# DaanVrancken/HubbardTN

Measured on AMD Instinct MI355X. Metric: DMRG sweep time (s) + GS energy/site, 1-band Hubbard L=64 chi=1024, lower is better.
Workload: dtype c128; 1 GPU; one-band Hubbard chain L=64 U/t=4, half filling, fZ2xSU(2)xU(1), two-site DMRG sweep (2L-3=125 bond updates) at chi=1024 (TensorKit dim units); model=one_band, L=64, chi=1024, krylovdim=30, parallelism=sector-parallel apply x1, backend=hip

## Files before the change

### hubbardtn_amd/csrc/htn_backend_hip.hip

```cpp
#include <dlfcn.h>

#include <map>
#include <mutex>

#include "htn_common.h"
#include "htn_core.h"

namespace {

__global__ __launch_bounds__(256) void k_scale_z(double2* __restrict__ x, int64_t n, double f) {
    for (int64_t j = (int64_t)blockIdx.x * blockDim.x + threadIdx.x; j < n; j += (int64_t)gridDim.x * blockDim.x) {
        const double2 v = x[j];
        x[j] = make_double2(v.x * f, v.y * f);
    }
}

__global__ __launch_bounds__(256) void k_copy_words(uint32_t* __restrict__ dst, const uint32_t* __restrict__ src, size_t n) {
    for (size_t j = (size_t)blockIdx.x * blockDim.x + threadIdx.x; j < n; j += (size_t)gridDim.x * blockDim.x) dst[j] = src[j];
    __threadfence_system();
}

struct Rccl {
    void* lib = nullptr;
    int (*GetUniqueId)(void*) = nullptr;
// ... 225 lines not shown
        if (nvec > 32) return htn::set_error("orthonormalise_rows: more than 32 rows");
        if (ensure_lan_scratch(htn_dots_scratch_elems(32) + 64)) return 1;
        double2* P = (double2*)Pv;
        double2* part = (double2*)lan_scratch;
        double2* coef = part + htn_dots_scratch_elems(32);
        double2* nrm = coef + 32;
        int k = 0;
        for (int r = 0; r < nvec; ++r) {
            double2* dst = P + (int64_t)k * n;
            if (r != k) HIP_TRY(hipMemcpyAsync(dst, P + (int64_t)r * n, sizeof(double2) * n, hipMemcpyDeviceToDevice, st));
            if (htn_dots_z(dst, n, 1, dst, n, nrm, part, st)) return 1;
            for (int pass = 0; pass < 2 && k > 0; ++pass) {
                if (htn_dots_z(P, n, k, dst, n, coef, part, st)) return 1;
                if (htn_axpys_z(dst, P, n, k, coef, -1.0, n, st)) return 1;
            }
            if (htn_dots_z(dst, n, 1, dst, n, nrm + 1, part, st)) return 1;
            double h[4];
            if (download(h, nrm, sizeof(h))) return 1;
            const double n0 = h[0], n1 = h[2];
            if (!(n0 > 0.0) || !(n1 > drop_tol * drop_tol * n0)) continue;
            if (htn_scale_inv_sqrt_z(dst, dst, nrm + 1, n, st)) return 1;
            ++k;
        }
        *kept = k;
        return 0;
    }
    int jacobi_svd(void* G, void* Vj, double* S, const htn_svd_block* desc_dev, const htn_svd_block* desc_host, int n_blocks,
                   int max_m, int max_sweeps, double tol, int32_t* info_dev, const htn_svd_opts* opts) override {
        fork_open = true;
        const int rc = htn_jacobi_svd_z(G, Vj, S, desc_dev, desc_host, n_blocks, max_m, max_sweeps, tol, info_dev, opts, st);
        fork_open = false;
        return rc;
    }
    int qr_blocks(void* A, void* R, const htn_qr_block* desc_dev, const htn_qr_block* desc_host, int n_blocks) override {
        return htn_qr_blocks_z(A, R, desc_dev, desc_host, n_blocks, st);
    }
    int block_trdots(const void* A, const void* B, const htn_trdot_item* items_dev, const htn_trdot_item* items_host, int n_items,
                     void* out, int n_out) override {
        (void)items_host;
        const int64_t need = htn_trdots_scratch_elems(n_items);
        if (need > trd_scratch_elems) {
            if (trd_scratch) HIP_TRY(hipFree(trd_scratch));
            trd_scratch = nullptr, trd_scratch_elems = 0;
            HIP_TRY(hipMalloc(&trd_scratch, sizeof(double2) * 2 * need));
            trd_scratch_elems = 2 * need;
            if (htn_debug_poison()) HIP_TRY(hipMemsetAsync(trd_scratch, 0xFF, sizeof(double2) * trd_scratch_elems, st));
        }
        return htn_block_trdots_z(A, B, items_dev, n_items, out, n_out, trd_scratch, st);
    }
    int batched_copy(void* dst, const void* src, const int32_t* idx, const double* scl, const htn_copy_item* items, int n_items,
                     double gscale) override {
        return htn_batched_copy_z(dst, src, idx, scl, items, n_items, gscale, st);
    }
    int scale(void* x, int64_t n, double f) override {
        if (n <= 0) return 0;
        const int grid = (int)std::min<int64_t>((n + 255) / 256, 2048);
        hipLaunchKernelGGL(k_scale_z, dim3(grid), dim3(256), 0, st, (double2*)x, n, f);
        HIP_TRY(hipGetLastError());
        return 0;
    }
    int set_comm(int rank, int world, const void* id) override {
        Rccl& r = rccl();
        if (!r.ok) return htn::set_error("htn_ctx_set_comm: librccl.so could not be loaded");
        if (comm) {
            r.CommDestroy(comm);
            comm = nullptr;
// ... 52 lines not shown
```

### hubbardtn_amd/csrc/htn_common.h

```cpp
#pragma once
#include <hip/hip_runtime.h>
#include <stdint.h>
#include <stdio.h>
#include <stdlib.h>
#include <string.h>

#include <map>
#include <memory>
#include <mutex>
#include <utility>

#include "hubbardtn_hip.h"

char* htn_err_buf();

static inline int htn_fail(const char* what, hipError_t e) {
    snprintf(htn_err_buf(), 512, "%s: %s", what, hipGetErrorString(e));
    return 1;
}
static inline int htn_fail_msg(const char* what) {
    snprintf(htn_err_buf(), 512, "%s", what);
    return 1;
}
#define fail htn_fail
// ... 5 lines not shown
    } while (0)

typedef double d4 __attribute__((ext_vector_type(4)));

static inline hipError_t htn_event_spin(hipEvent_t ev) {
    hipError_t e;
    while ((e = hipEventQuery(ev)) == hipErrorNotReady) __builtin_ia32_pause();
    return e;
}
static inline hipError_t htn_stream_spin(hipStream_t st) {
    static thread_local hipEvent_t evs[64] = {};
    int dev = 0;
    hipError_t e = hipGetDevice(&dev);
    if (e != hipSuccess) return e;
    if (dev < 0 || dev >= 64) return hipStreamSynchronize(st);
    if (!evs[dev] && (e = hipEventCreateWithFlags(&evs[dev], hipEventDisableTiming)) != hipSuccess) return e;
    if ((e = hipEventRecord(evs[dev], st)) != hipSuccess) return e;
    return htn_event_spin(evs[dev]);
}


static inline bool htn_env_flag(const char* name) {
    const char* v = getenv(name);
    return v && v[0] && v[0] != '0';
}
static inline bool htn_debug_poison() {
    static const bool on = htn_env_flag("HTN_DEBUG_POISON");
    return on;
}
static inline bool htn_debug_event_waits() {
    static const bool on = htn_env_flag("HTN_DEBUG_EVENT_WAITS");
    return on;
}

struct LanRecord {
    unsigned long long w[4];
};
__host__ __device__ __forceinline__ unsigned long long lan_rotl(unsigned long long x, int r) { return (x << r) | (x >> (64 - r)); }
__host__ __device__ __forceinline__ unsigned long long lan_check(unsigned long long w0, unsigned long long w1, unsigned long long w2,
                                                                 unsigned long long serial) {
    return serial ^ lan_rotl(w0, 13) ^ lan_rotl(w1, 29) ^ lan_rotl(w2, 47) ^ 0x9E3779B97F4A7C15ull;
}
#define HTN_DOT_BLOCKS 256
struct HtnGemmPublish {
    const double* norm_partial;
    const double2* c1;
    const double2* c2;
    LanRecord* rec_out;
    unsigned long long serial;
};
int htn_grouped_gemm_launch(const void* const* bufs_host, const htn_tile* tiles, int32_t n_tiles, const htn_seg* segs,
                            const HtnGemmPublish* pub, hipStream_t stream);

enum HtnBufKind {
    HTN_BUF_DEVICE,
    HTN_BUF_PINNED,
    HTN_BUF_MAPPED
};
struct HtnBuf {
    const HtnBufKind kind;
    const bool poison;
    void* p = nullptr;
    void* dev = nullptr;
    size_t cap = 0;
    explicit HtnBuf(HtnBufKind k, bool poison_new = true) : kind(k), poison(poison_new) {}
    HtnBuf(const HtnBuf&) = delete;
// ... 125 lines not shown
```

### hubbardtn_amd/csrc/htn_core.h

```cpp
#pragma once
#include <stdint.h>
#include <string.h>

#include <array>
#include <complex>
#include <memory>
#include <string>
#include <unordered_map>
#include <utility>
#include <vector>

#include "hubbardtn_hip.h"

namespace htn {

typedef std::complex<double> cplx;

enum { BUF_X = 0, BUF_Y, BUF_L, BUF_R, BUF_Z, BUF_S1, BUF_S2, BUF_AUX };

struct Sec {
    int32_t N, j;
};
inline bool operator<(const Sec& a, const Sec& b) { return a.N < b.N || (a.N == b.N && a.j < b.j); }
inline bool operator==(const Sec& a, const Sec& b) { return a.N == b.N && a.j == b.j; }
// ... 242 lines not shown
    bool has_cen = false;
    int64_t n_idx = 0;
};
void plan_finalize(const ThetaLayout& tl, const SvdPlan& sp, const std::vector<int>& keep, const SiteLayout& layA,
                   const SiteLayout& layB, bool right, int64_t offA, int64_t offB, FinalizePlan& out);

struct Backend {
    virtual ~Backend() {}
    virtual int kind() const = 0;
    virtual int activate() { return 0; }
    virtual void* alloc(size_t bytes) = 0;
    virtual void release(void* p) = 0;
    virtual int upload(void* dst, const void* src_host, size_t bytes) = 0;
    virtual int download(void* dst_host, const void* src, size_t bytes) = 0;
    virtual int zero(void* p, size_t bytes) = 0;
    virtual int sync() = 0;
    virtual int grouped_gemm(const void* const* bufs, const htn_tile* tiles, int32_t n_tiles, const htn_seg* segs) = 0;
    virtual int lanczos(const htn_gemm_launch* stages, int n_stages, int x_slot, int y_slot, void* V, int64_t n,
                        int krylovdim, double tol, int max_restart, int zero_y, htn_exchange2_fn exchange, void* user,
                        double* eig, int* n_matvec, double* residual, double* matvec_ms) = 0;
    virtual int lanczos_orth(const htn_gemm_launch* stages, int n_stages, int x_slot, int y_slot, void* V, int64_t n,
                             int krylovdim, double tol, int max_restart, int zero_y, htn_exchange2_fn exchange, void* user,
                             const void* Q, int n_frozen, double* eig, int* n_matvec, double* residual, double* matvec_ms);
    virtual int krylov_expm(const htn_gemm_launch* stages, int n_stages, int x_slot, int y_slot, void* V, int64_t n, int krylovdim,
                            double dt_re, double dt_im, double tol, int max_restart, int zero_y, htn_exchange2_fn exchange, void* user,
                            double* growth, double* alpha0, int* n_matvec, double* err, double* matvec_ms);
    virtual int orthonormalise_rows(void* P, int64_t n, int nvec, double drop_tol, int* kept);
    virtual int qr_blocks(void* A, void* R, const htn_qr_block* desc_dev, const htn_qr_block* desc_host, int n_blocks);
    virtual int block_trdots(const void* A, const void* B, const htn_trdot_item* items_dev, const htn_trdot_item* items_host,
                             int n_items, void* out, int n_out);
    virtual int jacobi_svd(void* G, void* Vj, double* S, const htn_svd_block* desc_dev, const htn_svd_block* desc_host,
                           int n_blocks, int max_m, int max_sweeps, double tol, int32_t* info_dev,
                           const htn_svd_opts* opts) = 0;
    virtual int batched_copy(void* dst, const void* src, const int32_t* idx, const double* scl,
                             const htn_copy_item* items_dev, int n_items, double gscale) = 0;
    virtual int scale(void* x, int64_t n, double f) = 0;
    virtual int set_comm(int rank, int world, const void* id) { return 1; }
    virtual bool has_comm() const { return false; }
    virtual int allreduce(void* y, int64_t n) { return 1; }
    bool timing = false;
};

void qr_blocks_host(cplx* A, cplx* R, const htn_qr_block* desc, int n_blocks);

int set_error(const char* fmt, ...);
char* err_buf();

}
```

### hubbardtn_amd/csrc/htn_engine.cpp

```cpp
#include <math.h>
#include <stdio.h>
#include <stdlib.h>

#include <algorithm>
#include <atomic>
#include <chrono>
#include <map>

#include "htn_core.h"
#include "htn_expm.h"

namespace htn {
Backend* make_backend(int backend, int device, void* stream);
}
using namespace htn;

namespace {
void tridiag_lowest_host(const std::vector<double>& alpha, const std::vector<double>& beta, double* eig, std::vector<double>& vec) {
    const int k = (int)alpha.size();
    auto count = [&](double x) {
        int cnt = 0;
        double d = 1.0;
        for (int i = 0; i < k; ++i) {
            d = (alpha[i] - x) - (i ? beta[i - 1] * beta[i - 1] / d : 0.0);
// ... 479 lines not shown
};
struct MeetC {
    std::vector<htn_trdot_item> items;
    DBufP items_dev;
};
struct OrthState {
    htn_mps* phi = nullptr;
    std::vector<OvlLayoutP> Llay, Rlay;
    std::vector<DView> Lbuf, Rbuf;
};
struct Solve {
    std::shared_ptr<ApplyC> ap;
    int64_t n = 0;
    double E = 0.0, res = 0.0, mv_ms = 0.0;
    int nmv = 0;
    double growth = 1.0;
};
struct BondWork {
    ThetaLayoutP tl;
    Solve sol;
    DView V, z, Qb;
    std::shared_ptr<SvdC> sc;
    DView G, Vj;
    DBufP S, idx;
    size_t s_elems = 0;
    std::vector<double> s_host;
    int jac_sweeps = 0;
    std::vector<int> lens, qd, counts;
    std::vector<std::vector<int>> order;
    std::vector<double> vals;
    double nrm = 0.0, tw = 0.0;
    BondP mid;
    double tA = 0.0, tB = 0.0, tC = 0.0, tD = 0.0;
};

}

struct htn_mps {
    std::atomic<int> refs{1};
    htn_ctx* ctx;
    htn_mpo* mpo_handle = nullptr;
    Backend* be;
    const Mpo* mpo;
    int L;
    std::vector<BondP> bonds;
    std::vector<SiteLayoutP> site_lay;
    std::vector<DView> site_buf;
    std::vector<EnvLayoutP> Llay, Rlay;
    std::vector<DView> Lbuf, Rbuf;
    std::unordered_map<std::string, std::shared_ptr<const void>> cache;
    int64_t hits = 0, misses = 0;
    double energy = 0.0;
    std::map<int, Spectrum> spectra;
    std::map<int, std::pair<std::pair<int, double>, double>> cut_hint;
    std::map<int, int> sweeps_hint;
    std::vector<int32_t> idx_host;
    std::vector<OrthState> orth;
    int orth_dropped = 0;
    int centre = 0;

    template <class T, class F>
    std::shared_ptr<T> cached(const std::string& key, F build) {
        auto it = cache.find(key);
        if (it != cache.end()) {
            ++hits;
            return std::const_pointer_cast<T>(std::static_pointer_cast<const T>(it->second));
// ... 61 lines not shown
        return cached<const ThetaLayout>(std::string("tl") + bl->key + "|" + br->key,
                                         [&] { return build_theta_layout(mpo->sym, bl, br); });
    }
    int gemm(const DevTasks& d, std::initializer_list<std::pair<int, const void*>> bufs) {
        if (d.ntiles == 0) return 0;
        if (ensure_ws(d.ws_slots)) return 1;
        const void* table[HTN_MAX_BUFS] = {nullptr};
        for (auto& kv : bufs) table[kv.first] = kv.second;
        table[HTN_BUF_WS] = ws.ptr();
        return be->grouped_gemm(table, d.tiles, d.ntiles, d.segs);
    }

    template <class C, class P>
    std::shared_ptr<C> compile2(std::shared_ptr<C> e, const P& p) {
        if (upload_tasks(p.t1, e->d1) || upload_tasks(p.t2, e->d2)) return nullptr;
        e->zsize = p.zsize;
        e->flops = p.t1.flops + p.t2.flops;
        return e;
    }
    int env_step(char side, int i);
    int left_env(int i) { return env_step('L', i); }
    int right_env(int i) { return env_step('R', i); }
    int ovl_step(char side, const htn_mps* ket, int i, const OvlLayoutP& inl, const DView& in, OvlLayoutP* outl, DView* out);
    int ovl_boundary(const htn_mps* ket, int b, OvlLayoutP* outl, DView* out);
    int ovl_project(const OrthState& o, int i, const ThetaLayout& tl, cplx* dst);
    int orth_attach(htn_mps* const* others, int n);
    void orth_detach();
    std::shared_ptr<ApplyC> compile_apply(ApplyPlan& p, bool deal_y);
    std::shared_ptr<ApplyC> make_apply(int i, const ThetaLayout& tl);
    std::shared_ptr<ApplyC> make_apply1(int i, const SiteLayout& lay);
    int apply_stages(const ApplyC& ap, const DView& L, const DView& R, const DView& z, htn_gemm_launch* stages);
    int apply_once(const ApplyC& ap, const DView& L, const DView& R, int64_t n, const void* x_host, void* y_host, bool exchange);
    int theta_into(int i, const ThetaLayout& tl, cplx* dst);
    int bond_solve(int i, bool optimise, const htn_sweep_opts& o, StageClock& clk, BondWork& w, const cplx* evolve_dt = nullptr);
    std::shared_ptr<SvdC> make_svd(int i, const ThetaLayout& tl, bool right);
    int bond_svd(int i, bool right, const htn_sweep_opts& o, BondWork& w);
    int bond_truncate(int i, const htn_sweep_opts& o, BondWork& w);
    int bond_finalise(int i, bool right, BondWork& w);
    int bond_advance(int i, bool right);
    void bond_spectrum(int i, const BondWork& w);
    void fill_stats(htn_bond_stats* st, int bond, int direction, const Solve& sol, int64_t env_elems, int jacobi_sweeps,
                    int64_t svd_flops, double trunc_weight, const StageClock& clk);
    int update_bond(int i, int direction, bool right, bool optimise, const htn_sweep_opts& o, htn_bond_stats* st,
                    const cplx* evolve_dt = nullptr, double* log_growth = nullptr);
    int sweep(const htn_sweep_opts& o, htn_bond_stats* st, double* E);
    int evolve_checks(const htn_sweep_opts& o, const char* who) const;
    int evolve_site(int i, cplx dt, const htn_sweep_opts& o, htn_bond_stats* st, double* log_growth);
    int tdvp2_sweep(cplx dt, const htn_sweep_opts& o, htn_bond_stats* st, double* E, double* log_norm);
    int set_mpo(htn_mpo* m);
    int relay(const SiteLayout& from, const cplx* src, const SiteLayout& to, cplx* dst);
    int update_site(int i, int direction, bool optimise, const htn_sweep_opts& o, htn_bond_stats* st);
    int sweep1(const htn_sweep_opts& o, htn_bond_stats* st, double* E);
    int correlator(const htn_corr_channel& ch, cplx* out_host, double* norm_host);
};

int htn_mps::env_step(char side, int i) {
    const bool left = side == 'L';
    const SiteLayout& lay = *site_lay[i];
    if (lay.kind != side)
        return left ? set_error("left_env: site %d is not in left layout", i) : set_error("right_env: site %d is not in right layout", i);
    const MpoSite& W = mpo->sites[i];
    const int from = left ? i : i + 1, to = left ? i + 1 : i;
    std::vector<EnvLayoutP>& elay = left ? Llay : Rlay;
    std::vector<DView>& ebuf = left ? Lbuf : Rbuf;
    auto c = cached<EnvC>(ikey(left ? "lenv" : "renv", i) + bonds[i]->key + "|" + bonds[i + 1]->key, [&]() -> std::shared_ptr<EnvC> {
        auto e = std::make_shared<EnvC>();
        e->lay = build_env_layout(mpo->sym, side, bonds[to], left ? W.right : W.left);
// ... 161 lines not shown

static int exchange_tramp(void* y, int64_t n, void* user) {
    htn_ctx* ctx = (htn_ctx*)user;
    if (ctx->exch) return ctx->exch(y, n, ctx->exch_user);
    return ctx->be->allreduce(y, n);
}

int htn_mps::apply_once(const ApplyC& ap, const DView& L, const DView& R, int64_t n, const void* x_host, void* y_host, bool exchange) {
    DView x = zalloc(n, false), y = zalloc(n, true), z = zalloc(ap.zsize, false);
    if (!x.base || !y.base || !z.base) return set_error("device allocation failed");
    if (be->upload(x.ptr(), x_host, sizeof(cplx) * n)) return 1;
    if (ap.has_z && gemm(ap.dz, {{BUF_X, x.ptr()}, {BUF_L, L.ptr()}, {BUF_Z, z.ptr()}})) return 1;
    if (gemm(ap.dy, {{BUF_X, x.ptr()}, {BUF_Y, y.ptr()}, {BUF_L, L.ptr()}, {BUF_R, R.ptr()}, {BUF_Z, z.ptr()}})) return 1;
    if (exchange && exchange_tramp(y.ptr(), n, ctx)) return set_error("htn_heff2_apply: exchange failed");
    return be->download(y_host, y.ptr(), sizeof(cplx) * n);
}

void htn_mps::fill_stats(htn_bond_stats* st, int bond, int direction, const Solve& sol, int64_t env_elems, int jacobi_sweeps,
                         int64_t svd_flops, double trunc_weight, const StageClock& clk) {
    memset(st, 0, sizeof(*st));
    st->bond = bond, st->direction = direction;
    st->n_matvec = sol.nmv, st->jacobi_sweeps = jacobi_sweeps;
    st->chi_full = (int32_t)bonds[bond]->dim_full(mpo->sym), st->multiplets = bonds[bond]->multiplets();
    st->n_tiles = sol.ap->ntiles, st->n_segs = sol.ap->nsegs;
    st->theta_size = sol.n;
    st->apply_flops = sol.ap->flops, st->apply_bytes = 16 * (2 * sol.n + env_elems), st->svd_flops = svd_flops;
    st->energy = sol.E, st->residual = sol.res, st->trunc_weight = trunc_weight;
    st->t_plan = clk.plan, st->t_lanczos = clk.lanczos, st->t_env = clk.env;
    st->t_total = now() - clk.t0;
    st->t_svd = clk.svd >= 0.0 ? clk.svd : st->t_total - clk.plan - clk.lanczos - clk.env;
    st->matvec_ms = sol.mv_ms > 0.0 ? sol.mv_ms : 0.0;
}

int htn_mps::bond_solve(int i, bool optimise, const htn_sweep_opts& o, StageClock& clk, BondWork& w, const cplx* evolve_dt) {
    w.tl = theta_layout(bonds[i], bonds[i + 2]);
    const ThetaLayout& tl = *w.tl;
    Solve& s = w.sol;
    const int64_t n = s.n = tl.size;
    const int kd = o.krylovdim;
    if (n <= 0) return set_error("htn_bond_update: empty two-site tensor on bond %d", i);
    w.V = zalloc((int64_t)(kd + 2) * n, false);
    if (!w.V.base) return set_error("device allocation of the Krylov basis failed (%lld elements)", (long long)((kd + 2) * n));
    if (theta_into(i, tl, w.V.ptr())) return 1;
    s.ap = make_apply(i, tl);
    if (!s.ap) return 1;
    w.z = zalloc(s.ap->zsize, false);
    htn_gemm_launch stages[2];
    const int ns = apply_stages(*s.ap, Lbuf[i], Rbuf[i + 2], w.z, stages);
    if (ns < 0) return 1;
    clk.plan = clk.lap();
    const bool shard = ctx->shard;
    int n_frozen = 0;
    if (!orth.empty() && optimise) {
        const int na = (int)orth.size();
        if (kd + na > 31)
            return set_error("htn_bond_update: krylovdim + attached states = %d + %d > 31 (row limit of the projected Lanczos step)", kd, na);
        w.Qb = zalloc((int64_t)na * n, false);
        if (!w.Qb.base) return set_error("device allocation of the projector rows failed");
        for (int k = 0; k < na; ++k)
            if (ovl_project(orth[k], i, tl, w.Qb.ptr() + (int64_t)k * n)) return 1;
        if (be->orthonormalise_rows(w.Qb.ptr(), n, na, 1e-12, &n_frozen)) return 1;
        orth_dropped = na - n_frozen;
    }
    if (evolve_dt) {
        if (be->krylov_expm(stages, ns, BUF_X, BUF_Y, w.V.ptr(), n, kd, evolve_dt->real(), evolve_dt->imag(), o.lanczos_tol, o.maxrestart, 0,
                            nullptr, ctx, &s.growth, &s.E, &s.nmv, &s.res, be->timing ? &s.mv_ms : nullptr))
            return 1;
    } else if (n_frozen > 0) {
        if (be->lanczos_orth(stages, ns, BUF_X, BUF_Y, w.V.ptr(), n, kd, o.lanczos_tol, o.maxrestart, shard ? 1 : 0,
                             shard ? exchange_tramp : nullptr, ctx, w.Qb.ptr(), n_frozen, &s.E, &s.nmv, &s.res,
                             be->timing ? &s.mv_ms : nullptr))
            return 1;
    } else if (be->lanczos(stages, ns, BUF_X, BUF_Y, w.V.ptr(), n, kd, optimise ? o.lanczos_tol : 1e300, o.maxrestart, shard ? 1 : 0,
                           shard ? exchange_tramp : nullptr, ctx, &s.E, &s.nmv, &s.res, be->timing ? &s.mv_ms : nullptr))
        return 1;
    clk.lanczos = clk.lap();
    return 0;
}

std::shared_ptr<SvdC> htn_mps::make_svd(int i, const ThetaLayout& tl, bool right) {
    return cached<SvdC>(std::string(right ? "svdR" : "svdL") + bonds[i]->key + "|" + bonds[i + 2]->key, [&]() -> std::shared_ptr<SvdC> {
        auto s = std::make_shared<SvdC>();
        if (plan_svd(tl, right, s->sp)) return nullptr;
        if (!(s->stage = upload_vec(be, s->sp.stage)) || !(s->desc = upload_vec(be, s->sp.desc))) return nullptr;
        if (ctx->world > 1) {
            const int nbk = (int)s->sp.mids.size();
            std::vector<int> ord(nbk);
            for (int b = 0; b < nbk; ++b) ord[b] = b;
            auto cost = [&](int b) { return (double)s->sp.desc[b].m * s->sp.desc[b].n * s->sp.desc[b].n; };
            std::stable_sort(ord.begin(), ord.end(), [&](int a, int b) { return cost(a) > cost(b); });
            std::vector<double> load(ctx->world, 0.0);
            std::vector<htn_copy_item> st_own;
            for (int b : ord) {
                int r = 0;
                for (int q = 1; q < ctx->world; ++q)
                    if (load[q] < load[r]) r = q;
                load[r] += cost(b);
                if (r == ctx->rank) {
                    s->own_desc.push_back(s->sp.desc[b]);
                    st_own.push_back(s->sp.stage[b]);
                }
            }
            s->n_own = (int)s->own_desc.size();
            if (s->n_own && (!(s->own_stage = upload_vec(be, st_own)) || !(s->own_desc_dev = upload_vec(be, s->own_desc)))) return nullptr;
        }
        return s;
    });
}

int htn_mps::bond_svd(int i, bool right, const htn_sweep_opts& o, BondWork& w) {
    w.sc = make_svd(i, *w.tl, right);
    if (!w.sc) return 1;
    const SvdC& sc = *w.sc;
    const SvdPlan& sp = sc.sp;
    const int nb = (int)sp.mids.size();
    w.G = zalloc(sp.g_size, false), w.Vj = zalloc(sp.v_size, false);
    w.s_elems = ((size_t)std::max<int64_t>(sp.s_size, 1) + 1) & ~(size_t)1;
    const size_t s_elems = w.s_elems, i_elems = (size_t)std::max(nb, 1);
    const size_t s_bytes = sizeof(double) * s_elems + sizeof(int32_t) * i_elems;
    w.S = dalloc(s_bytes);
    if (!w.G.base || !w.Vj.base || !w.S) return set_error("device allocation failed (SVD workspace)");
    int32_t* info_dev = (int32_t*)((double*)w.S->p + s_elems);
    const bool svd_shard = ctx->world > 1 && ctx->shard;
    const DBufP& stage = svd_shard ? sc.own_stage : sc.stage;
    const DBufP& desc_dev = svd_shard ? sc.own_desc_dev : sc.desc;
    const htn_svd_block* desc_host = svd_shard ? sc.own_desc.data() : sp.desc.data();
    const int n_run = svd_shard ? sc.n_own : nb;
    const bool run = n_run > 0 || !svd_shard;
    if (svd_shard) {
        if (be->zero(w.G.ptr(), sizeof(cplx) * (size_t)std::max<int64_t>(sp.g_size, 1))) return 1;
        if (be->zero(w.S->p, s_bytes)) return 1;
        if (sp.any_accumulate && be->zero(w.Vj.ptr(), sizeof(cplx) * (size_t)std::max<int64_t>(sp.v_size, 1))) return 1;
    }
    if (run && be->batched_copy(w.G.ptr(), w.V.ptr(), nullptr, nullptr, (const htn_copy_item*)stage->p, n_run, 1.0)) return 1;
    int32_t jac_used = 0;
    htn_svd_opts so = {o.svd_split_elems, 0, 0.0, &jac_used};
    {
        auto h = sweeps_hint.find(i + 1);
        if (h != sweeps_hint.end()) so.sweeps_hint = h->second;
    }
    if (o.rank_cut > 0.0) {
        double cut = 0.0;
        auto h = cut_hint.find(i + 1);
        if (h != cut_hint.end() && h->second.first.first == o.chi_full && h->second.first.second == o.cutoff)
            cut = o.rank_cut * h->second.second;
        so.rank_cut = std::max(cut, o.rank_cut * o.cutoff);
    }
    if (run && be->jacobi_svd(w.G.ptr(), w.Vj.ptr(), (double*)w.S->p, (const htn_svd_block*)desc_dev->p, desc_host, n_run, sp.max_m,
                              o.jacobi_max_sweeps, o.jacobi_tol, info_dev, &so))
        return 1;
    if (svd_shard) {
        if (exchange_tramp(w.G.ptr(), std::max<int64_t>(sp.g_size, 1), ctx)) return set_error("sharded SVD: exchange of the blocks failed");
        if (exchange_tramp(w.S->p, (int64_t)(s_elems / 2), ctx)) return set_error("sharded SVD: exchange of the singular values failed");
        if (sp.any_accumulate && exchange_tramp(w.Vj.ptr(), std::max<int64_t>(sp.v_size, 1), ctx)) return 1;
    }
    if (jac_used > 0) sweeps_hint[i + 1] = jac_used;
    w.tA = now();
    w.s_host.resize(s_elems + (i_elems + 1) / 2);
    if (be->download(w.s_host.data(), w.S->p, s_bytes)) return 1;
    w.tB = now();
    const int32_t* info_h = (const int32_t*)(w.s_host.data() + s_elems);
    for (int b = 0; b < n_run; ++b) {
        if (info_h[b] < 0) return set_error("Jacobi SVD did not converge (bond %d, block %d, %d sweeps)", i + 1, b, -info_h[b]);
        w.jac_sweeps = std::max(w.jac_sweeps, (int)info_h[b]);
    }
    return 0;
}

int htn_mps::bond_truncate(int i, const htn_sweep_opts& o, BondWork& w) {
    const SvdPlan& sp = w.sc->sp;
    const int nb = (int)sp.mids.size();
    w.lens.resize(nb), w.qd.resize(nb), w.order.resize(nb);
    w.vals.reserve((size_t)sp.s_size);
    std::vector<std::pair<double, int>> tmp;
    for (int b = 0; b < nb; ++b) {
        const int len = sp.desc[b].n;
        const double* sv = w.s_host.data() + sp.desc[b].s_off;
        w.lens[b] = len;
        w.qd[b] = mpo->sym.qdim(sp.mids[b]);
        tmp.resize(len);
// ... 87 lines not shown
}

int htn_mps::bond_advance(int i, bool right) {
    if (right ? left_env(i) : right_env(i + 1)) return 1;
    for (auto& os : orth)
        if (right ? ovl_step('L', os.phi, i, os.Llay[i], os.Lbuf[i], &os.Llay[i + 1], &os.Lbuf[i + 1])
                  : ovl_step('R', os.phi, i + 1, os.Rlay[i + 2], os.Rbuf[i + 2], &os.Rlay[i + 1], &os.Rbuf[i + 1]))
            return 1;
    return 0;
}

void htn_mps::bond_spectrum(int i, const BondWork& w) {
    const SvdPlan& sp = w.sc->sp;
    Spectrum spec;
    size_t p = 0;
    for (size_t b = 0; b < w.counts.size(); ++b) {
        if (w.counts[b] > 0) {
            spec.secs.push_back(sp.mids[b]);
            std::vector<double> v(w.counts[b]);
            const double f = 1.0 / w.nrm / sqrt((double)w.qd[b]);
            for (int k = 0; k < w.counts[b]; ++k) v[k] = w.vals[p + k] * f;
            spec.vals.push_back(std::move(v));
        }
        p += w.lens[b];
    }
    spectra[i + 1] = std::move(spec);
}

int htn_mps::update_bond(int i, int direction, bool right, bool optimise, const htn_sweep_opts& o, htn_bond_stats* st,
                         const cplx* evolve_dt, double* log_growth) {
    if (i < 0 || i + 1 >= L) return set_error("htn_bond_update: bond index %d out of range", i);
    StageClock clk(be, o.profile);
    BondWork w;
    if (bond_solve(i, optimise, o, clk, w, evolve_dt)) return 1;
    if (log_growth) *log_growth += log(w.sol.growth);
    const double t_svd0 = clk.last;
    if (bond_svd(i, right, o, w)) return 1;
    if (bond_truncate(i, o, w)) return 1;
    if (bond_finalise(i, right, w)) return 1;
    static const bool dbg_timers = getenv("HTN_DEBUG_HOST_TIMERS") != nullptr;
    if (dbg_timers)
        fprintf(stderr, "bond %d: svd call %.1f us, download %.1f, sort+truncate %.1f, finalize plan %.1f, enqueue %.1f  misses %lld hits %lld nvals %zu\n", i + 1,
                (w.tA - t_svd0) * 1e6, (w.tB - w.tA) * 1e6, (w.tC - w.tB) * 1e6, (w.tD - w.tC) * 1e6, (now() - w.tD) * 1e6, (long long)misses, (long long)hits, w.vals.size());
    clk.svd = clk.lap();
    if (bond_advance(i, right)) return 1;
    clk.env = clk.lap();
    energy = w.sol.E;
    centre = right ? i + 1 : i;
    bond_spectrum(i, w);
    if (st) fill_stats(st, i + 1, direction, w.sol, Llay[i]->size + Rlay[i + 2]->size, w.jac_sweeps, w.sc->sp.flops, w.tw, clk);
    return 0;
}

int htn_mps::sweep(const htn_sweep_opts& o, htn_bond_stats* st, double* E) {
    int k = 0;
    for (int i = 0; i < L - 1; ++i, ++k)
        if (update_bond(i, +1, i < L - 2, true, o, st ? st + k : nullptr)) return 1;
    for (int i = L - 3; i >= 0; --i, ++k)
        if (update_bond(i, -1, false, true, o, st ? st + k : nullptr)) return 1;
    if (E) *E = energy;
    return 0;
}

int htn_mps::relay(const SiteLayout& from, const cplx* src, const SiteLayout& to, cplx* dst) {
    auto rc = cached<RelayC>(std::string("relay") + from.kind + to.kind + from.bl->key + "|" + from.br->key, [&]() -> std::shared_ptr<RelayC> {
        std::vector<htn_copy_item> items;
        for (size_t q = 0; q < to.blocks.size(); ++q) {
// ... 1450 lines not shown
```

### hubbardtn_amd/csrc/htn_krylov.hip

```cpp
#include <math.h>

#include <chrono>
#include <vector>

#include "htn_common.h"
#include "htn_expm.h"

#define DOT_BLOCKS HTN_DOT_BLOCKS
#define DOT_THREADS 256
#define DOT_CHUNK 32

#define HTN_CH_DISPATCH(nvec, per, LAUNCH)          \
    do {                                            \
        if ((nvec) <= 4) LAUNCH(4, 256);            \
        else if ((nvec) <= 8) LAUNCH(8, 256);       \
        else if ((nvec) <= 12) LAUNCH(12, 256);     \
        else if ((nvec) <= 16) LAUNCH(16, 256);     \
        else if ((nvec) <= 20) LAUNCH(20, 256);     \
        else if ((nvec) <= 24) LAUNCH(24, 256);     \
        else if ((nvec) <= 28) LAUNCH(28, 256);     \
        else LAUNCH(32, 256);                       \
    } while (0)
static inline int64_t dot_slice(int64_t n) { return (n + DOT_BLOCKS - 1) / DOT_BLOCKS; }

// ... 378 lines not shown
                                                        const double2* __restrict__ nrm2, int64_t n) {
    const double s = 1.0 / sqrt(nrm2[0].x);
    for (int64_t j = (int64_t)blockIdx.x * blockDim.x + threadIdx.x; j < n; j += (int64_t)gridDim.x * blockDim.x) {
        const double2 v = src[j];
        dst[j] = make_double2(v.x * s, v.y * s);
    }
}

struct KrylovCoef {
    double2 c[DOT_CHUNK];
};
template <int CH, int TH>
__global__ __launch_bounds__(TH) void k_krylov_combine(double2* V, int64_t ldv, int nvec, int64_t n, const KrylovCoef kc) {
    for (int64_t j = (int64_t)blockIdx.x * TH + threadIdx.x; j < n; j += (int64_t)gridDim.x * TH) {
        double2 v[CH];
#pragma unroll
        for (int c = 0; c < CH; ++c) {
            const int i = c < nvec ? c : nvec - 1;
            v[c] = V[(int64_t)i * ldv + j];
        }
        double sr = 0.0, si = 0.0;
#pragma unroll
        for (int c = 0; c < CH; ++c) {
            sr += kc.c[c].x * v[c].x - kc.c[c].y * v[c].y;
            si += kc.c[c].x * v[c].y + kc.c[c].y * v[c].x;
        }
        V[j] = make_double2(sr, si);
    }
}

static inline int grid_for(int64_t n) {
    int64_t b = (n + 255) / 256;
    return (int)(b > 1024 ? 1024 : (b < 1 ? 1 : b));
}

static void launch_krylov_combine(double2* V, int64_t ldv, int nvec, int64_t n, const KrylovCoef& kc, hipStream_t st) {
#define HTN_KC(CHV, THV) hipLaunchKernelGGL((k_krylov_combine<CHV, THV>), dim3(grid_for(n)), dim3(THV), 0, st, V, ldv, nvec, n, kc)
    HTN_CH_DISPATCH(nvec, dot_slice(n), HTN_KC);
#undef HTN_KC
}

extern "C" int64_t htn_dots_scratch_elems(int32_t nvec) { return (int64_t)nvec * DOT_BLOCKS; }

extern "C" int htn_dots_z(const void* V, int64_t ldv, int32_t nvec, const void* w, int64_t n, void* out,
                          void* scratch, void* stream) {
    if (nvec <= 0) return 0;
    if (nvec > 64) return fail_msg("htn_dots_z: nvec > 64");
    launch_dots_partial((const double2*)V, ldv, nvec, (const double2*)w, n, (double2*)scratch, (hipStream_t)stream);
    hipLaunchKernelGGL(k_dots_reduce, dim3(nvec), dim3(64), 0, (hipStream_t)stream, (const double2*)scratch,
                       nvec, (double2*)out);
    HIP_TRY(hipGetLastError());
    return 0;
}

extern "C" int htn_axpys_z(void* w, const void* V, int64_t ldv, int32_t nvec, const void* coef, double sign,
                           int64_t n, void* stream) {
    if (nvec <= 0 || n <= 0) return 0;
    hipLaunchKernelGGL(k_axpys, dim3(grid_for(n)), dim3(256), 0, (hipStream_t)stream, (double2*)w, (const double2*)V,
                       ldv, nvec, (const double2*)coef, sign, n);
    HIP_TRY(hipGetLastError());
    return 0;
}

extern "C" int htn_scale_inv_sqrt_z(void* dst, const void* src, const void* nrm2, int64_t n, void* stream) {
    if (n <= 0) return 0;
    hipLaunchKernelGGL(k_scale_inv_sqrt, dim3(grid_for(n)), dim3(256), 0, (hipStream_t)stream, (double2*)dst,
// ... 79 lines not shown
    ~LanRes() {
        if (device >= 0) (void)hipSetDevice(device);
        if (h_rec) (void)hipHostFree(h_rec);
        if (h_y) (void)hipHostFree(h_y);
        if (have_events)
            for (int i = 0; i < LAN_SLOTS; ++i) {
                (void)hipEventDestroy(ev_done[i]);
                (void)hipEventDestroy(ev_mv0[i]);
                (void)hipEventDestroy(ev_mv1[i]);
            }
    }
};
HtnStreamRegistry<LanRes> g_lan_res;

int lan_res_get(hipStream_t st, LanRes** out) {
    return g_lan_res.get(st, out, [](LanRes& r) -> int {
        HIP_TRY(hipHostMalloc((void**)&r.h_rec, sizeof(LanRecord) * LAN_SLOTS, hipHostMallocMapped | hipHostMallocCoherent));
        memset(r.h_rec, 0, sizeof(LanRecord) * LAN_SLOTS);
        HIP_TRY(hipHostGetDevicePointer((void**)&r.d_rec, r.h_rec, 0));
        HIP_TRY(hipHostMalloc((void**)&r.h_y, sizeof(double2) * LAN_SLOTS, hipHostMallocDefault));
        for (int i = 0; i < LAN_SLOTS; ++i) {
            HIP_TRY(hipEventCreateWithFlags(&r.ev_done[i], hipEventDisableTiming));
            HIP_TRY(hipEventCreate(&r.ev_mv0[i]));
            HIP_TRY(hipEventCreate(&r.ev_mv1[i]));
        }
        r.have_events = true;
        return 0;
    });
}
}

void htn_krylov_release_stream(hipStream_t st) { g_lan_res.release(st); }

static int lanczos_run(const htn_gemm_launch* stages, int32_t n_stages, int32_t x_slot, int32_t y_slot,
                       void* Vv, int64_t n, int32_t krylovdim, double tol, int32_t max_restart,
                       void* scratch, int32_t zero_y, htn_exchange2_fn exchange, void* user,
                       double* eig_host, int32_t* n_matvec_host, double* residual_host,
                       double* matvec_ms_host, void* stream_v, const double2* Q, int nf, htn_expm::Expm* ex = nullptr) {
    hipStream_t st = (hipStream_t)stream_v;
    const int kd = krylovdim;
    const int kt = kd + nf;
    double2* V = (double2*)Vv;
    double2* partial = (double2*)scratch;
    double2* partial2 = partial + (int64_t)(kt + 1) * DOT_BLOCKS;
    double2* c1 = partial2 + (int64_t)(kt + 1) * DOT_BLOCKS;
    double2* c2 = c1 + (kt + 1);
    double2* ycoef = c2 + (kt + 1);
    double* norm_partial = (double*)(ycoef + (kt + 1));

    LanRes* R = nullptr;
    if (lan_res_get(st, &R)) return 1;
    const bool event_waits = htn_debug_event_waits();
    static const bool full_first_pass = htn_env_flag("HTN_LANCZOS_FULL_FIRST_PASS");

    bool timed_step[LAN_SLOTS] = {false};
    unsigned long long step_serial[LAN_SLOTS] = {0};
    const bool solo = ex && ex->dt_re == 0.0 && ex->dt_im == 0.0;
    auto matvec = [&](double2* x, double2* y, const HtnGemmPublish* pub) -> int {
        if (zero_y) HIP_TRY(hipMemsetAsync(y, 0, sizeof(double2) * n, st));
        bool published = pub == nullptr;
        for (int s = 0; s < n_stages; ++s) {
            const void* bufs[HTN_MAX_BUFS];
            for (int b = 0; b < HTN_MAX_BUFS; ++b) bufs[b] = stages[s].bufs[b];
            bufs[x_slot] = x;
            bufs[y_slot] = y;
            const bool here = !published && stages[s].n_tiles > 0;
            if (htn_grouped_gemm_launch(bufs, stages[s].tiles, stages[s].n_tiles, stages[s].segs, here ? pub : nullptr, st)) return 1;
            published |= here;
        }
        if (!published)
            hipLaunchKernelGGL(k_publish_record, dim3(1), dim3(64), 0, st, pub->norm_partial, pub->c1, pub->c2, pub->rec_out, pub->serial);
        if (exchange && exchange(y, n, user)) return fail_msg("htn_lanczos_z: the exchange hook reported a failure");
        return 0;
    };
    auto enqueue_step = [&](int j, bool first) -> int {
        double2* vj = V + (int64_t)j * n;
        double2* w = V + (int64_t)(j + 1) * n;
        const bool timed = matvec_ms_host && (R->sample % 8) == 0;
        timed_step[j] = timed;
        ++R->sample;
        step_serial[j] = ++R->serial;
        HtnGemmPublish pub = {nullptr, nullptr, nullptr, nullptr, 0ull};
// ... 32 lines not shown
    auto wait_step = [&](int j, double* a1, double* a2, double* nn) -> int {
        if (event_waits) {
            HIP_TRY(hipEventSynchronize(R->ev_done[j]));
            if (!read_record(j, a1, a2, nn)) return fail_msg("htn_lanczos_z: the step's event completed but its record does not validate");
            return 0;
        }
        for (unsigned spins = 1;; ++spins) {
            if (read_record(j, a1, a2, nn)) return 0;
            __builtin_ia32_pause();
            if ((spins & 0xffff) == 0) {
                const hipError_t q = hipStreamQuery(st);
                if (q == hipSuccess)
                    return read_record(j, a1, a2, nn) ? 0 : fail_msg("htn_lanczos_z: the stream drained without producing the step's record");
                if (q != hipErrorNotReady) return fail("hipStreamQuery", q);
            }
        }
    };

    auto project_out = [&](double2* w) {
        for (int pass = 0; pass < 2; ++pass) {
            launch_dots_partial(Q, n, nf, w, n, partial, st);
            launch_axpy_norm(w, Q, n, nf, partial, c1, -1, -1.0, n, norm_partial, st);
        }
    };
    if (nf > 0) project_out(V);
    else
    hipLaunchKernelGGL(k_norm_partial, dim3(DOT_BLOCKS), dim3(DOT_THREADS), 0, st, V, n, norm_partial);
    hipLaunchKernelGGL(k_scale_by_norm, dim3(grid_for(n)), dim3(DOT_THREADS), 0, st, V, V, norm_partial, n,
                       (LanRecord*)nullptr, (const double2*)nullptr, (const double2*)nullptr, 0ull);
    double mv_ms = 0.0;
    int nmv = 0, n_timed = 0;
    static const bool dbg_timers = getenv("HTN_DEBUG_HOST_TIMERS") != nullptr;
    auto now_us = [] { return std::chrono::duration<double, std::micro>(std::chrono::steady_clock::now().time_since_epoch()).count(); };
    double t_enq = 0.0, t_wait = 0.0, t_host = 0.0;
    const double t_begin = now_us();
    double theta = 0.0, res = 0.0, beta = 0.0, amax = 0.0;
    std::vector<double> y;
    for (int restart = 0; restart <= max_restart; ++restart) {
        std::vector<double> alphas, betas;
        if (ex) ex->begin_cycle();
        double tq = now_us();
        if (enqueue_step(0, true)) return 1;
        t_enq += now_us() - tq;
        ++nmv;
        for (int j = 0; j < kd; ++j) {
            if (j + 1 < kd && !solo) {
                tq = now_us();
                if (enqueue_step(j + 1, false)) return 1;
                t_enq += now_us() - tq;
                ++nmv;
            }
            double a1 = 0.0, a2 = 0.0, nn = 0.0;
            tq = now_us();
            if (wait_step(j, &a1, &a2, &nn)) return 1;
            t_wait += now_us() - tq;
            tq = now_us();
            if (timed_step[j]) {
                float ms = 0.f;
                HIP_TRY(htn_event_spin(R->ev_mv1[j]));
                HIP_TRY(hipEventElapsedTime(&ms, R->ev_mv0[j], R->ev_mv1[j]));
                mv_ms += ms;
                ++n_timed;
            }
            const double alpha = a1 + a2;
            if (!(alpha == alpha) || !(nn == nn)) return fail_msg("htn_lanczos_z: NaN in the tridiagonal coefficients (operator or start vector not finite)");
            beta = sqrt(nn > 0.0 ? nn : 0.0);
            if (ex) {
                bool bad = false;
                const bool stop = ex->step(alpha, beta, kd, &bad);
                if (bad) return fail_msg("htn_krylov_expm_z: the QL iteration of the tridiagonal matrix did not converge");
                t_host += now_us() - tq;
                if (stop) break;
                continue;
            }
            alphas.push_back(alpha);
            tridiag_lowest(alphas, betas, &theta, y);
            res = fabs(beta * y.back());
            amax = std::max(amax, std::max(fabs(alpha), beta));
            t_host += now_us() - tq;
            if (res < tol || beta < 1e-14 * std::max(amax, 1e-300) || j == kd - 1) break;
            betas.push_back(beta);
        }
        if (ex) {
            if (!ex->converged && restart == max_restart) {
                HIP_TRY(htn_stream_spin(st));
                snprintf(htn_err_buf(), 512, "htn_krylov_expm_z: not converged after %d restart(s) of krylovdim %d: fraction %.3e of dt remains "
                         "(estimate %.3e, tol %.3e)", max_restart, kd, ex->remaining, ex->est, tol);
                return 1;
            }
            if (!ex->finish()) {
                HIP_TRY(htn_stream_spin(st));
                return fail_msg("htn_krylov_expm_z: no fraction of the step down to 2^-60 meets the tolerance");
            }
            const int m = (int)ex->c.size();
            KrylovCoef kc;
            for (int i = 0; i < DOT_CHUNK; ++i) kc.c[i] = i < m ? make_double2(ex->c[i].real(), ex->c[i].imag()) : make_double2(0.0, 0.0);
            launch_krylov_combine(V, n, m, n, kc, st);
            if (ex->remaining == 0.0) break;
            continue;
        }
        HIP_TRY(htn_stream_spin(st));
        const int k = (int)y.size();
        for (int i = 0; i < k; ++i) R->h_y[i] = make_double2(y[i], 0.0);
        HIP_TRY(hipMemcpyAsync(ycoef, R->h_y, sizeof(double2) * k, hipMemcpyHostToDevice, st));
        double2* xrow = V + (int64_t)(kd + 1) * n;
        HIP_TRY(hipMemsetAsync(xrow, 0, sizeof(double2) * n, st));
        hipLaunchKernelGGL(k_axpys, dim3(grid_for(n)), dim3(256), 0, st, xrow, V, n, k, ycoef, 1.0, n);
        if (nf > 0) project_out(xrow);
        else
        hipLaunchKernelGGL(k_norm_partial, dim3(DOT_BLOCKS), dim3(DOT_THREADS), 0, st, xrow, n, norm_partial);
        hipLaunchKernelGGL(k_scale_by_norm, dim3(grid_for(n)), dim3(DOT_THREADS), 0, st, V, xrow, norm_partial, n,
                           (LanRecord*)nullptr, (const double2*)nullptr, (const double2*)nullptr, 0ull);
        HIP_TRY(htn_stream_spin(st));
        if (res < tol || beta < 1e-14 * std::max(amax, 1e-300)) break;
    }
    HIP_TRY(hipGetLastError());
    if (dbg_timers)
        fprintf(stderr, "lanczos n=%lld: %d matvecs in %.1f us: enqueue %.1f, waiting for records %.1f, tridiagonal %.1f\n", (long long)n, nmv,
                now_us() - t_begin, t_enq, t_wait, t_host);
    *eig_host = ex ? ex->alpha0 : theta;
    *n_matvec_host = nmv;
    *residual_host = ex ? ex->err_total : res;
    if (matvec_ms_host) *matvec_ms_host = n_timed ? mv_ms * nmv / n_timed : -1.0;
    return 0;
}

extern "C" int htn_lanczos_z(const htn_gemm_launch* stages, int32_t n_stages, int32_t x_slot, int32_t y_slot,
                             void* Vv, int64_t n, int32_t krylovdim, double tol, int32_t max_restart,
                             void* scratch, int32_t zero_y, htn_exchange2_fn exchange, void* user,
                             double* eig_host, int32_t* n_matvec_host, double* residual_host,
                             double* matvec_ms_host, void* stream_v) {
    if (krylovdim < 2 || krylovdim + 1 > DOT_CHUNK) return fail_msg("htn_lanczos_z: krylovdim must be in 2..31");
    return lanczos_run(stages, n_stages, x_slot, y_slot, Vv, n, krylovdim, tol, max_restart, scratch, zero_y, exchange, user,
                       eig_host, n_matvec_host, residual_host, matvec_ms_host, stream_v, nullptr, 0);
}

extern "C" int htn_lanczos_orth_z(const htn_gemm_launch* stages, int32_t n_stages, int32_t x_slot, int32_t y_slot,
                                  void* Vv, int64_t n, int32_t krylovdim, double tol, int32_t max_restart,
                                  void* scratch, int32_t zero_y, htn_exchange2_fn exchange, void* user,
                                  double* eig_host, int32_t* n_matvec_host, double* residual_host,
                                  double* matvec_ms_host, const void* Q, int32_t n_frozen, void* stream_v) {
    if (n_frozen < 0 || (n_frozen > 0 && !Q)) return fail_msg("htn_lanczos_orth_z: n_frozen rows need a device pointer Q");
    if (krylovdim < 2 || krylovdim + n_frozen + 1 > DOT_CHUNK)
        return fail_msg("htn_lanczos_orth_z: krylovdim >= 2 and krylovdim + n_frozen <= 31 required");
    return lanczos_run(stages, n_stages, x_slot, y_slot, Vv, n, krylovdim, tol, max_restart, scratch, zero_y, exchange, user,
                       eig_host, n_matvec_host, residual_host, matvec_ms_host, stream_v, (const double2*)Q, n_frozen);
}

extern "C" int htn_krylov_combine_z(void* V, int64_t ldv, int32_t nvec, const double* coef_host, int64_t n, void* stream) {
    if (nvec < 1 || nvec > DOT_CHUNK) return fail_msg("htn_krylov_combine_z: nvec must be in 1..32");
    if (!V || !coef_host || n < 0 || ldv < n) return fail_msg("htn_krylov_combine_z: bad arguments (V, coef_host, 0 <= n <= ldv)");
    if (n == 0) return 0;
// ... 26 lines not shown
```

Baseline: 407.6 ms.

## Overlap SVD workspace setup with Lanczos and fuse Ritz vector combine

Registers a callback so that the bond SVD setup (plan construction, device allocations, option hints) runs on the host while the first Lanczos matvec is in flight, instead of after the solve. It also replaces the host-to-device coefficient copy, memset and axpys sequence for the Ritz vector with a single kernel that takes its coefficients as kernel arguments. Device allocations inside the callback could introduce implicit synchronisation, and an error in the callback is only reported after the solver returns. A legacy environment flag restores the old path.

```diff
diff --git a/hubbardtn_amd/csrc/htn_backend_hip.hip b/hubbardtn_amd/csrc/htn_backend_hip.hip
--- a/hubbardtn_amd/csrc/htn_backend_hip.hip
+++ b/hubbardtn_amd/csrc/htn_backend_hip.hip
@@ -281,6 +281,9 @@
         fork_open = false;
         return rc;
     }
+    void while_solving(void (*fn)(void*), void* user) override {
+        if (!htn_bond_legacy_setup()) htn_krylov_while_solving(fn, user);
+    }
     int qr_blocks(void* A, void* R, const htn_qr_block* desc_dev, const htn_qr_block* desc_host, int n_blocks) override {
         return htn_qr_blocks_z(A, R, desc_dev, desc_host, n_blocks, st);
     }
diff --git a/hubbardtn_amd/csrc/htn_common.h b/hubbardtn_amd/csrc/htn_common.h
--- a/hubbardtn_amd/csrc/htn_common.h
+++ b/hubbardtn_amd/csrc/htn_common.h
@@ -61,6 +61,12 @@
     static const bool on = htn_env_flag("HTN_DEBUG_EVENT_WAITS");
     return on;
 }
+static inline bool htn_bond_legacy_setup() {
+    static const bool on = htn_env_flag("HTN_BOND_LEGACY_SETUP");
+    return on;
+}
+
+void htn_krylov_while_solving(void (*fn)(void*), void* user);
 
 struct LanRecord {
     unsigned long long w[4];
diff --git a/hubbardtn_amd/csrc/htn_core.h b/hubbardtn_amd/csrc/htn_core.h
--- a/hubbardtn_amd/csrc/htn_core.h
+++ b/hubbardtn_amd/csrc/htn_core.h
@@ -298,6 +298,7 @@
     virtual int jacobi_svd(void* G, void* Vj, double* S, const htn_svd_block* desc_dev, const htn_svd_block* desc_host,
                            int n_blocks, int max_m, int max_sweeps, double tol, int32_t* info_dev,
                            const htn_svd_opts* opts) = 0;
+    virtual void while_solving(void (*fn)(void*), void* user) { (void)fn, (void)user; }
     virtual int batched_copy(void* dst, const void* src, const int32_t* idx, const double* scl,
                              const htn_copy_item* items_dev, int n_items, double gscale) = 0;
     virtual int scale(void* x, int64_t n, double f) = 0;
diff --git a/hubbardtn_amd/csrc/htn_engine.cpp b/hubbardtn_amd/csrc/htn_engine.cpp
--- a/hubbardtn_amd/csrc/htn_engine.cpp
+++ b/hubbardtn_amd/csrc/htn_engine.cpp
@@ -535,6 +535,17 @@
     double nrm = 0.0, tw = 0.0;
     BondP mid;
     double tA = 0.0, tB = 0.0, tC = 0.0, tD = 0.0;
+    bool svd_set = false;
+    int svd_set_rc = 0;
+    htn_svd_opts so = {0, 0, 0.0, nullptr};
+    int32_t jac_used = 0;
+};
+struct SvdSetupCall {
+    htn_mps* psi;
+    int i;
+    bool right;
+    const htn_sweep_opts* o;
+    BondWork* w;
 };
 
 }
@@ -662,7 +673,8 @@
     int apply_stages(const ApplyC& ap, const DView& L, const DView& R, const DView& z, htn_gemm_launch* stages);
     int apply_once(const ApplyC& ap, const DView& L, const DView& R, int64_t n, const void* x_host, void* y_host, bool exchange);
     int theta_into(int i, const ThetaLayout& tl, cplx* dst);
-    int bond_solve(int i, bool optimise, const htn_sweep_opts& o, StageClock& clk, BondWork& w, const cplx* evolve_dt = nullptr);
+    int bond_solve(int i, bool right, bool optimise, const htn_sweep_opts& o, StageClock& clk, BondWork& w, const cplx* evolve_dt = nullptr);
+    int bond_svd_setup(int i, bool right, const htn_sweep_opts& o, BondWork& w);
     std::shared_ptr<SvdC> make_svd(int i, const ThetaLayout& tl, bool right);
     int bond_svd(int i, bool right, const htn_sweep_opts& o, BondWork& w);
     int bond_truncate(int i, const htn_sweep_opts& o, BondWork& w);
@@ -890,7 +902,7 @@
     st->matvec_ms = sol.mv_ms > 0.0 ? sol.mv_ms : 0.0;
 }
 
-int htn_mps::bond_solve(int i, bool optimise, const htn_sweep_opts& o, StageClock& clk, BondWork& w, const cplx* evolve_dt) {
+int htn_mps::bond_solve(int i, bool right, bool optimise, const htn_sweep_opts& o, StageClock& clk, BondWork& w, const cplx* evolve_dt) {
     w.tl = theta_layout(bonds[i], bonds[i + 2]);
     const ThetaLayout& tl = *w.tl;
     Solve& s = w.sol;
@@ -920,18 +932,25 @@
         if (be->orthonormalise_rows(w.Qb.ptr(), n, na, 1e-12, &n_frozen)) return 1;
         orth_dropped = na - n_frozen;
     }
+    SvdSetupCall setup = {this, i, right, &o, &w};
+    be->while_solving([](void* u) {
+        SvdSetupCall& q = *(SvdSetupCall*)u;
+        q.w->svd_set_rc = q.psi->bond_svd_setup(q.i, q.right, *q.o, *q.w);
+    }, &setup);
+    int rc = 0;
     if (evolve_dt) {
-        if (be->krylov_expm(stages, ns, BUF_X, BUF_Y, w.V.ptr(), n, kd, evolve_dt->real(), evolve_dt->imag(), o.lanczos_tol, o.maxrestart, 0,
-                            nullptr, ctx, &s.growth, &s.E, &s.nmv, &s.res, be->timing ? &s.mv_ms : nullptr))
-            return 1;
+        rc = be->krylov_expm(stages, ns, BUF_X, BUF_Y, w.V.ptr(), n, kd, evolve_dt->real(), evolve_dt->imag(), o.lanczos_tol, o.maxrestart, 0,
+                             nullptr, ctx, &s.growth, &s.E, &s.nmv, &s.res, be->timing ? &s.mv_ms : nullptr);
     } else if (n_frozen > 0) {
-        if (be->lanczos_orth(stages, ns, BUF_X, BUF_Y, w.V.ptr(), n, kd, o.lanczos_tol, o.maxrestart, shard ? 1 : 0,
-                             shard ? exchange_tramp : nullptr, ctx, w.Qb.ptr(), n_frozen, &s.E, &s.nmv, &s.res,
-                             be->timing ? &s.mv_ms : nullptr))
-            return 1;
-    } else if (be->lanczos(stages, ns, BUF_X, BUF_Y, w.V.ptr(), n, kd, optimise ? o.lanczos_tol : 1e300, o.maxrestart, shard ? 1 : 0,
-                           shard ? exchange_tramp : nullptr, ctx, &s.E, &s.nmv, &s.res, be->timing ? &s.mv_ms : nullptr))
-        return 1;
+        rc = be->lanczos_orth(stages, ns, BUF_X, BUF_Y, w.V.ptr(), n, kd, o.lanczos_tol, o.maxrestart, shard ? 1 : 0,
+                              shard ? exchange_tramp : nullptr, ctx, w.Qb.ptr(), n_frozen, &s.E, &s.nmv, &s.res,
+                              be->timing ? &s.mv_ms : nullptr);
+    } else
+        rc = be->lanczos(stages, ns, BUF_X, BUF_Y, w.V.ptr(), n, kd, optimise ? o.lanczos_tol : 1e300, o.maxrestart, shard ? 1 : 0,
+                         shard ? exchange_tramp : nullptr, ctx, &s.E, &s.nmv, &s.res, be->timing ? &s.mv_ms : nullptr);
+    be->while_solving(nullptr, nullptr);
+    if (rc) return 1;
+    if (w.svd_set_rc) return 1;
     clk.lanczos = clk.lap();
     return 0;
 }
@@ -966,7 +985,9 @@
     });
 }
 
-int htn_mps::bond_svd(int i, bool right, const htn_sweep_opts& o, BondWork& w) {
+int htn_mps::bond_svd_setup(int i, bool right, const htn_sweep_opts& o, BondWork& w) {
+    if (w.svd_set) return 0;
+    w.svd_set = true;
     w.sc = make_svd(i, *w.tl, right);
     if (!w.sc) return 1;
     const SvdC& sc = *w.sc;
@@ -978,6 +999,28 @@
     const size_t s_bytes = sizeof(double) * s_elems + sizeof(int32_t) * i_elems;
     w.S = dalloc(s_bytes);
     if (!w.G.base || !w.Vj.base || !w.S) return set_error("device allocation failed (SVD workspace)");
+    w.so = {o.svd_split_elems, 0, 0.0, &w.jac_used};
+    {
+        auto h = sweeps_hint.find(i + 1);
+        if (h != sweeps_hint.end()) w.so.sweeps_hint = h->second;
+    }
+    if (o.rank_cut > 0.0) {
+        double cut = 0.0;
+        auto h = cut_hint.find(i + 1);
+        if (h != cut_hint.end() && h->second.first.first == o.chi_full && h->second.first.second == o.cutoff)
+            cut = o.rank_cut * h->second.second;
+        w.so.rank_cut = std::max(cut, o.rank_cut * o.cutoff);
+    }
+    return 0;
+}
+
+int htn_mps::bond_svd(int i, bool right, const htn_sweep_opts& o, BondWork& w) {
+    if (bond_svd_setup(i, right, o, w)) return 1;
+    const SvdC& sc = *w.sc;
+    const SvdPlan& sp = sc.sp;
+    const int nb = (int)sp.mids.size();
+    const size_t s_elems = w.s_elems, i_elems = (size_t)std::max(nb, 1);
+    const size_t s_bytes = sizeof(double) * s_elems + sizeof(int32_t) * i_elems;
     int32_t* info_dev = (int32_t*)((double*)w.S->p + s_elems);
     const bool svd_shard = ctx->world > 1 && ctx->shard;
     const DBufP& stage = svd_shard ? sc.own_stage : sc.stage;
@@ -991,19 +1034,8 @@
         if (sp.any_accumulate && be->zero(w.Vj.ptr(), sizeof(cplx) * (size_t)std::max<int64_t>(sp.v_size, 1))) return 1;
     }
     if (run && be->batched_copy(w.G.ptr(), w.V.ptr(), nullptr, nullptr, (const htn_copy_item*)stage->p, n_run, 1.0)) return 1;
-    int32_t jac_used = 0;
-    htn_svd_opts so = {o.svd_split_elems, 0, 0.0, &jac_used};
-    {
-        auto h = sweeps_hint.find(i + 1);
-        if (h != sweeps_hint.end()) so.sweeps_hint = h->second;
-    }
-    if (o.rank_cut > 0.0) {
-        double cut = 0.0;
-        auto h = cut_hint.find(i + 1);
-        if (h != cut_hint.end() && h->second.first.first == o.chi_full && h->second.first.second == o.cutoff)
-            cut = o.rank_cut * h->second.second;
-        so.rank_cut = std::max(cut, o.rank_cut * o.cutoff);
-    }
+    htn_svd_opts& so = w.so;
+    int32_t& jac_used = w.jac_used;
     if (run && be->jacobi_svd(w.G.ptr(), w.Vj.ptr(), (double*)w.S->p, (const htn_svd_block*)desc_dev->p, desc_host, n_run, sp.max_m,
                               o.jacobi_max_sweeps, o.jacobi_tol, info_dev, &so))
         return 1;
@@ -1157,7 +1189,7 @@
     if (i < 0 || i + 1 >= L) return set_error("htn_bond_update: bond index %d out of range", i);
     StageClock clk(be, o.profile);
     BondWork w;
-    if (bond_solve(i, optimise, o, clk, w, evolve_dt)) return 1;
+    if (bond_solve(i, right, optimise, o, clk, w, evolve_dt)) return 1;
     if (log_growth) *log_growth += log(w.sol.growth);
     const double t_svd0 = clk.last;
     if (bond_svd(i, right, o, w)) return 1;
diff --git a/hubbardtn_amd/csrc/htn_krylov.hip b/hubbardtn_amd/csrc/htn_krylov.hip
--- a/hubbardtn_amd/csrc/htn_krylov.hip
+++ b/hubbardtn_amd/csrc/htn_krylov.hip
@@ -434,6 +434,23 @@
 static inline int grid_for(int64_t n) {
     int64_t b = (n + 255) / 256;
     return (int)(b > 1024 ? 1024 : (b < 1 ? 1 : b));
+}
+
+__global__ __launch_bounds__(256) void k_ritz_combine(double2* __restrict__ x, const double2* __restrict__ V, int64_t ldv, int nvec,
+                                                      const KrylovCoef kc, double sign, int64_t n) {
+    for (int64_t j = (int64_t)blockIdx.x * blockDim.x + threadIdx.x; j < n; j += (int64_t)gridDim.x * blockDim.x) {
+        double sr = 0.0, si = 0.0;
+        for (int i = 0; i < nvec; ++i) {
+            const double2 c = kc.c[i];
+            const double2 v = V[(int64_t)i * ldv + j];
+            sr += c.x * v.x - c.y * v.y;
+            si += c.x * v.y + c.y * v.x;
+        }
+        double2 r = make_double2(0.0, 0.0);
+        r.x += sign * sr;
+        r.y += sign * si;
+        x[j] = r;
+    }
 }
 
 static void launch_krylov_combine(double2* V, int64_t ldv, int nvec, int64_t n, const KrylovCoef& kc, hipStream_t st) {
@@ -579,6 +596,18 @@
 
 void htn_krylov_release_stream(hipStream_t st) { g_lan_res.release(st); }
 
+namespace {
+struct HtnWhileSolving {
+    void (*fn)(void*) = nullptr;
+    void* user = nullptr;
+};
+thread_local HtnWhileSolving g_while_solving;
+}
+void htn_krylov_while_solving(void (*fn)(void*), void* user) {
+    g_while_solving.fn = fn;
+    g_while_solving.user = user;
+}
+
 static int lanczos_run(const htn_gemm_launch* stages, int32_t n_stages, int32_t x_slot, int32_t y_slot,
                        void* Vv, int64_t n, int32_t krylovdim, double tol, int32_t max_restart,
                        void* scratch, int32_t zero_y, htn_exchange2_fn exchange, void* user,
@@ -595,6 +624,8 @@
     double2* ycoef = c2 + (kt + 1);
     double* norm_partial = (double*)(ycoef + (kt + 1));
 
+    HtnWhileSolving beside = g_while_solving;
+    g_while_solving = HtnWhileSolving();
     LanRes* R = nullptr;
     if (lan_res_get(st, &R)) return 1;
     const bool event_waits = htn_debug_event_waits();
@@ -693,7 +724,7 @@
     int nmv = 0, n_timed = 0;
     static const bool dbg_timers = getenv("HTN_DEBUG_HOST_TIMERS") != nullptr;
     auto now_us = [] { return std::chrono::duration<double, std::micro>(std::chrono::steady_clock::now().time_since_epoch()).count(); };
-    double t_enq = 0.0, t_wait = 0.0, t_host = 0.0;
+    double t_enq = 0.0, t_wait = 0.0, t_host = 0.0, t_beside = 0.0;
     const double t_begin = now_us();
     double theta = 0.0, res = 0.0, beta = 0.0, amax = 0.0;
     std::vector<double> y;
@@ -712,6 +743,13 @@
                 ++nmv;
             }
             double a1 = 0.0, a2 = 0.0, nn = 0.0;
+            if (beside.fn) {
+                tq = now_us();
+                const HtnWhileSolving b = beside;
+                beside = HtnWhileSolving();
+                b.fn(b.user);
+                t_beside += now_us() - tq;
+            }
             tq = now_us();
             if (wait_step(j, &a1, &a2, &nn)) return 1;
             t_wait += now_us() - tq;
@@ -762,11 +800,17 @@
         }
         HIP_TRY(htn_stream_spin(st));
         const int k = (int)y.size();
-        for (int i = 0; i < k; ++i) R->h_y[i] = make_double2(y[i], 0.0);
-        HIP_TRY(hipMemcpyAsync(ycoef, R->h_y, sizeof(double2) * k, hipMemcpyHostToDevice, st));
         double2* xrow = V + (int64_t)(kd + 1) * n;
-        HIP_TRY(hipMemsetAsync(xrow, 0, sizeof(double2) * n, st));
-        hipLaunchKernelGGL(k_axpys, dim3(grid_for(n)), dim3(256), 0, st, xrow, V, n, k, ycoef, 1.0, n);
+        if (htn_bond_legacy_setup()) {
+            for (int i = 0; i < k; ++i) R->h_y[i] = make_double2(y[i], 0.0);
+            HIP_TRY(hipMemcpyAsync(ycoef, R->h_y, sizeof(double2) * k, hipMemcpyHostToDevice, st));
+            HIP_TRY(hipMemsetAsync(xrow, 0, sizeof(double2) * n, st));
+            hipLaunchKernelGGL(k_axpys, dim3(grid_for(n)), dim3(256), 0, st, xrow, V, n, k, ycoef, 1.0, n);
+        } else {
+            KrylovCoef kc;
+            for (int i = 0; i < DOT_CHUNK; ++i) kc.c[i] = make_double2(i < k ? y[i] : 0.0, 0.0);
+            hipLaunchKernelGGL(k_ritz_combine, dim3(grid_for(n)), dim3(256), 0, st, xrow, (const double2*)V, n, k, kc, 1.0, n);
+        }
         if (nf > 0) project_out(xrow);
         else
         hipLaunchKernelGGL(k_norm_partial, dim3(DOT_BLOCKS), dim3(DOT_THREADS), 0, st, xrow, n, norm_partial);
@@ -777,8 +821,8 @@
     }
     HIP_TRY(hipGetLastError());
     if (dbg_timers)
-        fprintf(stderr, "lanczos n=%lld: %d matvecs in %.1f us: enqueue %.1f, waiting for records %.1f, tridiagonal %.1f\n", (long long)n, nmv,
-                now_us() - t_begin, t_enq, t_wait, t_host);
+        fprintf(stderr, "lanczos n=%lld: %d matvecs in %.1f us: enqueue %.1f, waiting for records %.1f, tridiagonal %.1f, caller's set-up %.1f\n",
+                (long long)n, nmv, now_us() - t_begin, t_enq, t_wait, t_host, t_beside);
     *eig_host = ex ? ex->alpha0 : theta;
     *n_matvec_host = nmv;
     *residual_host = ex ? ex->err_total : res;
```

Result: no change. 404.7 ms (median of 5 runs) (-0.7%).
